# FengDushuo/BBBP-Multi-Modal-Deep-Ensemble-Framework

Measured on AMD Instinct MI355X. Metric: molecules/sec fwd+bwd (3-branch ensemble, B=512), higher is better.
Workload: dtype f32; 1 GPU; MixedInputModel F=167 (MACCS) + 3x128x128 image, 6-layer encoder + 2-stage CNN + fusion + BN head; forward + MSE + backward + fused AdamW, train mode (dropout 0.1); global_batch=512, per_gpu_batch=512, parallelism=dp1, input=device-resident

## Files before the change

bbbp-multi-modal-deep-ensemble-framework_amd/csrc/head.hip:

```cpp
#include "common.h"
#include "bbbp_hip.h"
#include "head_sync.h"

namespace {

constexpr int ROWS = 16;
constexpr int NTH = 512;
constexpr int NW = NTH / 64;
constexpr int COMB = 256, FHID = 128, NHEADS = 4, H1 = 256, H2 = 128, H3 = 64;
constexpr int LD = COMB + 4;
typedef float f32x4g __attribute__((ext_vector_type(4), aligned(4)));
static_assert(NTH >= H1, "one thread per BatchNorm column");

struct HeadParams {
    const float* comb;
    const float* fw1[NHEADS]; const float* fb1[NHEADS]; const float* fw2[NHEADS]; const float* fb2[NHEADS];
    const float* w0; const float* b0;
    const float* gamma; const float* beta; float* running_mean; float* running_var;
    const float* w3; const float* b3;
    const float* w5; const float* b5;
    const float* w7; const float* b7;
    float* hid; float* attn; float* fused; float* h; float* hb; float* bn_mean; float* bn_rstd; float* h2; float* h3; float* out;
    float* partial;
    int B, training;
    float eps, momentum;
    int concat;
    int world, rank;
};

template <int NCH>
__device__ __forceinline__ void load_b(f32x4 (&bf)[NCH], const float* Wrow ) {
#pragma unroll
    for (int c = 0; c < NCH; ++c) { f32x4g v = *reinterpret_cast<const f32x4g*>(Wrow + 16 * c); bf[c] = f32x4{v[0], v[1], v[2], v[3]}; }
}
template <int NCH>
__device__ __forceinline__ f32x4 mma_tile(const f32x4 (&af)[NCH], const f32x4 (&bf)[NCH]) {
    f32x4 acc0 = {0.f, 0.f, 0.f, 0.f}, acc1 = {0.f, 0.f, 0.f, 0.f};
#pragma unroll
    for (int c = 0; c < NCH; ++c)
#pragma unroll
        for (int j = 0; j < 4; j += 2) {
            acc0 = __builtin_amdgcn_mfma_f32_16x16x4f32(af[c][j], bf[c][j], acc0, 0, 0, 0);
            acc1 = __builtin_amdgcn_mfma_f32_16x16x4f32(af[c][j + 1], bf[c][j + 1], acc1, 0, 0, 0);
        }
    return acc0 + acc1;
}

template <int NCH>
__device__ __forceinline__ void load_a(f32x4 (&af)[NCH], const float* s, int ld, int lane) {
    const int i = lane & 15, kq = lane >> 4;
#pragma unroll
    for (int c = 0; c < NCH; ++c) af[c] = *reinterpret_cast<const f32x4*>(s + i * ld + 16 * c + 4 * kq);
}

__device__ __forceinline__ float sum16(float v) {
    v += __shfl_xor(v, 1); v += __shfl_xor(v, 2); v += __shfl_xor(v, 4); v += __shfl_xor(v, 8);
    return v;
}

__global__ __launch_bounds__(NTH) void head_a_kernel(HeadParams p) {
    __shared__ __attribute__((aligned(16))) float sC[ROWS * LD];
    __shared__ float sLogit[NW][NHEADS][ROWS];
    __shared__ float sP[ROWS][NHEADS];
    const int t = threadIdx.x, lane = t & 63, wave = t >> 6;
    const int q = lane & 15, kq = lane >> 4;
    const int r0 = blockIdx.x * ROWS, nrows = min(ROWS, p.B - r0);
    for (int idx = t; idx < ROWS * (COMB / 4); idx += NTH) {
        const int r = idx / (COMB / 4), c4 = idx % (COMB / 4);
        f32x4 v = {0.f, 0.f, 0.f, 0.f};
        if (r < nrows) v = *reinterpret_cast<const f32x4*>(p.comb + (long)(r0 + r) * COMB + c4 * 4);
        *reinterpret_cast<f32x4*>(sC + r * LD + c4 * 4) = v;
    }
    __syncthreads();
    f32x4 af[COMB / 16];
    load_a<COMB / 16>(af, sC, LD, lane);
    float lg[NHEADS][4];
    f32x4 bf[2][COMB / 16];
    const int n = wave * 16 + q;
    if (p.concat) {
        load_b<COMB / 16>(bf[0], p.w0 + (long)n * COMB + 4 * kq);
    } else {
    load_b<COMB / 16>(bf[0], p.fw1[0] + (long)n * COMB + 4 * kq);
#pragma unroll
    for (int h = 0; h < NHEADS; ++h) {
        if (h + 1 < NHEADS) load_b<COMB / 16>(bf[(h + 1) & 1], p.fw1[h + 1] + (long)n * COMB + 4 * kq);
        else load_b<COMB / 16>(bf[(h + 1) & 1], p.w0 + (long)n * COMB + 4 * kq);
        f32x4 acc = mma_tile<COMB / 16>(af, bf[h & 1]);
        const float b = p.fb1[h][n], w2 = p.fw2[h][n];
#pragma unroll
        for (int r = 0; r < 4; ++r) {
            const int row = 4 * kq + r;
            const float v = tanhf(acc[r] + b);
            if (row < nrows) p.hid[((long)h * p.B + r0 + row) * FHID + n] = v;
            lg[h][r] = sum16(v * w2);
        }
    }
    if (q == 0) {
#pragma unroll
        for (int h = 0; h < NHEADS; ++h)
#pragma unroll
            for (int r = 0; r < 4; ++r) sLogit[wave][h][4 * kq + r] = lg[h][r];
    }
    __syncthreads();
    if (t < ROWS) {
        float a[NHEADS], m = -INFINITY;
#pragma unroll
        for (int h = 0; h < NHEADS; ++h) {
            float z = 0.f;
#pragma unroll
            for (int w = 0; w < NW; ++w) z += sLogit[w][h][t];
            a[h] = z + p.fb2[h][0];
            m = fmaxf(m, a[h]);
        }
        float den = 0.f;
#pragma unroll
        for (int h = 0; h < NHEADS; ++h) { a[h] = __expf(a[h] - m); den += a[h]; }
#pragma unroll
        for (int h = 0; h < NHEADS; ++h) {
            a[h] /= den;
            sP[t][h] = a[h];
            if (t < nrows) p.attn[(long)(r0 + t) * NHEADS + h] = a[h];
        }
    }
    __syncthreads();
    for (int idx = t; idx < ROWS * COMB; idx += NTH) {
        const int r = idx / COMB, c = idx % COMB;
        const float x = sC[r * LD + c];
        float s = 0.f;
#pragma unroll
        for (int h = 0; h < NHEADS; ++h) s += sP[r][h] * x;
        sC[r * LD + c] = s;
        if (r < nrows) p.fused[(long)(r0 + r) * COMB + c] = s;
    }
    __syncthreads();
    load_a<COMB / 16>(af, sC, LD, lane);
    }
#pragma unroll
    for (int tt = 0; tt < 2; ++tt) {
        const int n0 = (wave + NW * tt) * 16 + q;
        if (tt == 0) load_b<COMB / 16>(bf[1], p.w0 + (long)((wave + NW) * 16 + q) * COMB + 4 * kq);
        f32x4 acc = mma_tile<COMB / 16>(af, bf[tt & 1]);
        const float b = p.b0[n0];
        float v[4], s = 0.f;
#pragma unroll
        for (int r = 0; r < 4; ++r) {
            const int row = 4 * kq + r;
            v[r] = fmaxf(acc[r] + b, 0.f);
            if (row < nrows) { p.h[(long)(r0 + row) * H1 + n0] = v[r]; s += v[r]; }
        }
        s += __shfl_xor(s, 16); s += __shfl_xor(s, 32);
        const float mean = s / nrows;
        float m2 = 0.f;
#pragma unroll
        for (int r = 0; r < 4; ++r) if (4 * kq + r < nrows) { const float d = v[r] - mean; m2 += d * d; }
        m2 += __shfl_xor(m2, 16); m2 += __shfl_xor(m2, 32);
        if (kq == 0) {
            const long slot = (long)p.rank * gridDim.x + blockIdx.x;
            p.partial[(slot * 2 + 0) * H1 + n0] = mean;
            p.partial[(slot * 2 + 1) * H1 + n0] = m2;
        }
    }
}

__global__ __launch_bounds__(NTH) void head_b_kernel(HeadParams p) {
    __shared__ __attribute__((aligned(16))) float sA[ROWS * LD];
    __shared__ __attribute__((aligned(16))) float sB[ROWS * (H2 + 4)];
    __shared__ __attribute__((aligned(16))) float sD[ROWS * (H3 + 4)];
    __shared__ float sMean[H1], sRstd[H1];
    const int t = threadIdx.x, lane = t & 63, wave = t >> 6;
    const int q = lane & 15, kq = lane >> 4;
    const int r0 = blockIdx.x * ROWS, nrows = min(ROWS, p.B - r0);
    const int nblocks = (p.B + ROWS - 1) / ROWS;
    f32x4 bf3[H1 / 16];
    load_b<H1 / 16>(bf3, p.w3 + (long)(wave * 16 + q) * H1 + 4 * kq);
    if (t < H1) {
        const int c = t;
        float mean, rstd;
        if (p.training) {
            float na = 0.f, ma = 0.f, m2a = 0.f;
            for (int b = 0; b < nblocks * p.world; ++b) {
                const float nb = (float)min(ROWS, p.B - (b % nblocks) * ROWS);
                const float mb = p.partial[((long)b * 2 + 0) * H1 + c], m2b = p.partial[((long)b * 2 + 1) * H1 + c];
                const float d = mb - ma, n = na + nb;
                ma += d * (nb / n);
                m2a += m2b + d * d * (na * nb / n);
                na = n;
            }
            const float nall = (float)p.B * (float)p.world;
            const float var = m2a / nall;
            mean = ma; rstd = rsqrtf(var + p.eps);
            if (blockIdx.x == 0) {
                p.running_mean[c] = (1.f - p.momentum) * p.running_mean[c] + p.momentum * mean;
                p.running_var[c] = (1.f - p.momentum) * p.running_var[c] + p.momentum * var * (nall / (nall - 1.f));
            }
        } else {
            mean = p.running_mean[c]; rstd = rsqrtf(p.running_var[c] + p.eps);
        }
        sMean[c] = mean; sRstd[c] = rstd;
        if (blockIdx.x == 0) { p.bn_mean[c] = mean; p.bn_rstd[c] = rstd; }
    }
    __syncthreads();
    for (int idx = t; idx < ROWS * H1; idx += NTH) {
        const int r = idx / H1, c = idx % H1;
        float v = 0.f;
        if (r < nrows) {
            v = (p.h[(long)(r0 + r) * H1 + c] - sMean[c]) * sRstd[c] * p.gamma[c] + p.beta[c];
            p.hb[(long)(r0 + r) * H1 + c] = v;
        }
        sA[r * LD + c] = v;
    }
    __syncthreads();
    {
        f32x4 af[H1 / 16];
        load_a<H1 / 16>(af, sA, LD, lane);
        const int n = wave * 16 + q;
        f32x4 acc = mma_tile<H1 / 16>(af, bf3);
        const float b = p.b3[n];
#pragma unroll
        for (int r = 0; r < 4; ++r) {
            const int row = 4 * kq + r;
            const float v = fmaxf(acc[r] + b, 0.f);
            sB[row * (H2 + 4) + n] = v;
            if (row < nrows) p.h2[(long)(r0 + row) * H2 + n] = v;
        }
    }
    __syncthreads();
    if (wave < H3 / 16) {
        f32x4 af[H2 / 16], bf[H2 / 16];
        const int n = wave * 16 + q;
        load_b<H2 / 16>(bf, p.w5 + (long)n * H2 + 4 * kq);
        load_a<H2 / 16>(af, sB, H2 + 4, lane);
        f32x4 acc = mma_tile<H2 / 16>(af, bf);
        const float b = p.b5[n];
#pragma unroll
        for (int r = 0; r < 4; ++r) {
            const int row = 4 * kq + r;
            const float v = fmaxf(acc[r] + b, 0.f);
            sD[row * (H3 + 4) + n] = v;
            if (row < nrows) p.h3[(long)(r0 + row) * H3 + n] = v;
        }
    }
    __syncthreads();
    if (wave == 0) {
        const int row = lane >> 2, part = lane & 3;
        float s = 0.f;
#pragma unroll
        for (int k = 0; k < H3 / 4; ++k) s += sD[row * (H3 + 4) + part * (H3 / 4) + k] * p.w7[part * (H3 / 4) + k];
        s += __shfl_xor(s, 1); s += __shfl_xor(s, 2);
        if (part == 0 && row < nrows) p.out[r0 + row] = s + p.b7[0];
    }
}

struct HeadBwdParams {
    const float* dout;
    const float* comb; const float* hid; const float* attn; const float* h; const float* h2; const float* h3;
    const float* bn_mean; const float* bn_rstd; const float* gamma;
    const float* fw1[NHEADS]; const float* fw2[NHEADS];
    const float* w0; const float* w3; const float* w5; const float* w7;
    float* dh3; float* dh2; float* dhb; float* dh; float* dlogit; float* dpre; float* dcomb;
    float* dgamma; float* dbeta;
    float* partial;
    int B, training;
    int world, rank;
};

typedef float f32x2g __attribute__((ext_vector_type(2), aligned(4)));

template <int K, int T>
__device__ __forceinline__ void mma_kmajor(f32x4 (&acc)[T], const float* sA, int lda, const float* W, int ldw, int colbase, int lane) {
    const int q = lane & 15, kq = lane >> 4;
    const float* wcol = W + colbase + T * q;
#pragma unroll 4
    for (int c = 0; c < K / 16; ++c) {
        const f32x4 a = *reinterpret_cast<const f32x4*>(sA + q * lda + 16 * c + 4 * kq);
#pragma unroll
        for (int j = 0; j < 4; ++j) {
            const float* wr = wcol + (long)(16 * c + 4 * kq + j) * ldw;
            if constexpr (T == 2) {
                const f32x2g b = *reinterpret_cast<const f32x2g*>(wr);
                acc[0] = __builtin_amdgcn_mfma_f32_16x16x4f32(a[j], b[0], acc[0], 0, 0, 0);
                acc[1] = __builtin_amdgcn_mfma_f32_16x16x4f32(a[j], b[1], acc[1], 0, 0, 0);
            } else {
                acc[0] = __builtin_amdgcn_mfma_f32_16x16x4f32(a[j], wr[0], acc[0], 0, 0, 0);
            }
        }
    }
}

constexpr int LD2 = H2 + 4, LD3 = H3 + 4, LDP = FHID + 4;

__global__ __launch_bounds__(NTH) void head_bwd_a_kernel(HeadBwdParams p) {
    __shared__ __attribute__((aligned(16))) float sD3[ROWS * LD3];
    __shared__ __attribute__((aligned(16))) float sD2[ROWS * LD2];
    __shared__ float sPa[4][H1], sPb[4][H1];
    const int t = threadIdx.x, lane = t & 63, wave = t >> 6;
    const int q = lane & 15, kq = lane >> 4;
    const int r0 = blockIdx.x * ROWS, nrows = min(ROWS, p.B - r0);
    for (int idx = t; idx < ROWS * H3; idx += NTH) {
        const int r = idx / H3, c = idx % H3;
        float v = 0.f;
        if (r < nrows) {
            v = p.h3[(long)(r0 + r) * H3 + c] > 0.f ? p.dout[r0 + r] * p.w7[c] : 0.f;
            p.dh3[(long)(r0 + r) * H3 + c] = v;
        }
        sD3[r * LD3 + c] = v;
    }
    __syncthreads();
    {
        f32x4 acc[1] = {{0.f, 0.f, 0.f, 0.f}};
        mma_kmajor<H3, 1>(acc, sD3, LD3, p.w5, H2, wave * 16, lane);
        const int n = wave * 16 + q;
#pragma unroll
        for (int r = 0; r < 4; ++r) {
            const int row = 4 * kq + r;
            float v = 0.f;
            if (row < nrows) {
                v = p.h2[(long)(r0 + row) * H2 + n] > 0.f ? acc[0][r] : 0.f;
                p.dh2[(long)(r0 + row) * H2 + n] = v;
            }
            sD2[row * LD2 + n] = v;
        }
    }
    __syncthreads();
    {
        f32x4 acc[2] = {{0.f, 0.f, 0.f, 0.f}, {0.f, 0.f, 0.f, 0.f}};
        mma_kmajor<H2, 2>(acc, sD2, LD2, p.w3, H1, wave * 32, lane);
#pragma unroll
        for (int u = 0; u < 2; ++u) {
            const int n = wave * 32 + 2 * q + u;
            const float mu = p.bn_mean[n], rs = p.bn_rstd[n];
            float pa = 0.f, pb = 0.f;
#pragma unroll
            for (int r = 0; r < 4; ++r) {
                const int row = 4 * kq + r;
                if (row < nrows) {
                    const float g = acc[u][r];
                    p.dhb[(long)(r0 + row) * H1 + n] = g;
                    pa += g * (p.h[(long)(r0 + row) * H1 + n] - mu) * rs;
                    pb += g;
                }
            }
            sPa[kq][n] = pa; sPb[kq][n] = pb;
        }
    }
    __syncthreads();
    if (t < H1) {
        const long slot = (long)p.rank * gridDim.x + blockIdx.x;
        p.partial[(slot * 2 + 0) * H1 + t] = ((sPa[0][t] + sPa[1][t]) + sPa[2][t]) + sPa[3][t];
        p.partial[(slot * 2 + 1) * H1 + t] = ((sPb[0][t] + sPb[1][t]) + sPb[2][t]) + sPb[3][t];
    }
}

__global__ __launch_bounds__(NTH) void head_bwd_c_kernel(HeadBwdParams p) {
    __shared__ __attribute__((aligned(16))) float sX[ROWS * LD];
    __shared__ __attribute__((aligned(16))) float sP[NHEADS * ROWS * LDP];
    __shared__ float sSa[H1], sSb[H1];
    const int t = threadIdx.x, lane = t & 63, wave = t >> 6;
    const int q = lane & 15, kq = lane >> 4;
    const int r0 = blockIdx.x * ROWS, nrows = min(ROWS, p.B - r0);
    const int nblocks = (p.B + ROWS - 1) / ROWS;
    if (t < H1) {
        float sa = 0.f, sb = 0.f, la = 0.f, lb = 0.f;
        for (int b = 0; b < nblocks * p.world; ++b) {
            const float va = p.partial[((long)b * 2 + 0) * H1 + t], vb = p.partial[((long)b * 2 + 1) * H1 + t];
            sa += va; sb += vb;
            if (b / nblocks == p.rank) { la += va; lb += vb; }
        }
        sSa[t] = sa; sSb[t] = sb;
        if (blockIdx.x == 0) { p.dgamma[t] = la; p.dbeta[t] = lb; }
    }
    __syncthreads();
    for (int idx = t; idx < ROWS * H1; idx += NTH) {
        const int r = idx / H1, c = idx % H1;
        float v = 0.f;
        if (r < nrows) {
            const float d = p.dhb[(long)(r0 + r) * H1 + c], xv = p.h[(long)(r0 + r) * H1 + c];
            const float g = p.gamma[c], mu = p.bn_mean[c], rs = p.bn_rstd[c];
            const float nall = (float)p.B * (float)p.world;
            v = p.training ? g * rs * (d - sSb[c] / nall - (xv - mu) * rs * (sSa[c] / nall)) : d * g * rs;
            v = xv > 0.f ? v : 0.f;
            p.dh[(long)(r0 + r) * H1 + c] = v;
        }
        sX[r * LD + c] = v;
    }
    __syncthreads();
    f32x4 df[2] = {{0.f, 0.f, 0.f, 0.f}, {0.f, 0.f, 0.f, 0.f}};
    mma_kmajor<H1, 2>(df, sX, LD, p.w0, COMB, wave * 32, lane);
    __syncthreads();
#pragma unroll
    for (int u = 0; u < 2; ++u)
#pragma unroll
        for (int r = 0; r < 4; ++r) sX[(4 * kq + r) * LD + wave * 32 + 2 * q + u] = df[u][r];
    __syncthreads();
#pragma unroll
    for (int rr = 0; rr < 2; ++rr) {
        const int r = wave * 2 + rr;
        const bool live = r < nrows;
        float a[NHEADS], asum = 0.f;
#pragma unroll
        for (int hh = 0; hh < NHEADS; ++hh) { a[hh] = live ? p.attn[(long)(r0 + r) * NHEADS + hh] : 0.f; asum += a[hh]; }
        float tt = 0.f;
#pragma unroll
        for (int c = lane; c < COMB; c += 64) {
            const float g = sX[r * LD + c];
            tt += live ? g * p.comb[(long)(r0 + r) * COMB + c] : 0.f;
            sX[r * LD + c] = g * asum;
        }
#pragma unroll
        for (int o = 32; o > 0; o >>= 1) tt += __shfl_xor(tt, o);
#pragma unroll
        for (int hh = 0; hh < NHEADS; ++hh) {
            const float dl = a[hh] * (tt - tt * asum);
            if (lane == 0 && live) p.dlogit[(long)hh * p.B + r0 + r] = dl;
#pragma unroll
            for (int c = lane; c < FHID; c += 64) {
                float v = 0.f;
                if (live) {
                    const float y = p.hid[((long)hh * p.B + r0 + r) * FHID + c];
                    v = dl * p.fw2[hh][c] * (1.f - y * y);
                    p.dpre[((long)hh * p.B + r0 + r) * FHID + c] = v;
                }
                sP[(hh * ROWS + r) * LDP + c] = v;
            }
        }
    }
    __syncthreads();
    f32x4 acc[2] = {{0.f, 0.f, 0.f, 0.f}, {0.f, 0.f, 0.f, 0.f}};
#pragma unroll
    for (int hh = 0; hh < NHEADS; ++hh) mma_kmajor<FHID, 2>(acc, sP + hh * ROWS * LDP, LDP, p.fw1[hh], COMB, wave * 32, lane);
#pragma unroll
    for (int u = 0; u < 2; ++u) {
        const int n = wave * 32 + 2 * q + u;
#pragma unroll
        for (int r = 0; r < 4; ++r) {
            const int row = 4 * kq + r;
            if (row < nrows) {
                const float v = acc[u][r] + sX[row * LD + n];
                p.dcomb[(long)(r0 + row) * COMB + n] = p.comb[(long)(r0 + row) * COMB + n] > 0.f ? v : 0.f;
            }
        }
    }
}

}

int bbbp_head_forward_fused(hipStream_t st, const float* comb, const float* const* fw1, const float* const* fb1,
                            const float* const* fw2, const float* const* fb2, const float* w0, const float* b0, const float* gamma,
                            const float* beta, float* running_mean, float* running_var, const float* w3, const float* b3,
                            const float* w5, const float* b5, const float* w7, const float* b7, float* hid, float* attn, float* fused,
                            float* h, float* hb, float* bn_mean, float* bn_rstd, float* h2, float* h3, float* out, float* partial,
                            int B, int training, int concat) {
    return bbbp_head_forward_fused_sync(st, comb, fw1, fb1, fw2, fb2, w0, b0, gamma, beta, running_mean, running_var, w3, b3, w5, b5, w7, b7,
                                        hid, attn, fused, h, hb, bn_mean, bn_rstd, h2, h3, out, partial, B, training, concat, nullptr);
}

int bbbp_head_forward_fused_sync(hipStream_t st, const float* comb, const float* const* fw1, const float* const* fb1,
                                 const float* const* fw2, const float* const* fb2, const float* w0, const float* b0, const float* gamma,
                                 const float* beta, float* running_mean, float* running_var, const float* w3, const float* b3,
                                 const float* w5, const float* b5, const float* w7, const float* b7, float* hid, float* attn, float* fused,
                                 float* h, float* hb, float* bn_mean, float* bn_rstd, float* h2, float* h3, float* out, float* partial,
                                 int B, int training, int concat, const bbbp_head_sync* sync) {
    const int world = sync ? sync->world : 1, rank = sync ? sync->rank : 0;
    BBBP_CHECK_ARG(B >= 1, "head: empty batch");
    BBBP_CHECK_ARG(world >= 1 && rank >= 0 && rank < world, "head: rank %d of %d", rank, world);
    BBBP_CHECK_ARG(!(training && (long)B * world <= 1), "Expected more than 1 value per channel when training, got input size [%d, %d]", B, H1);
    HeadParams p;
    p.comb = comb;
    for (int i = 0; i < NHEADS; ++i) { p.fw1[i] = fw1[i]; p.fb1[i] = fb1[i]; p.fw2[i] = fw2[i]; p.fb2[i] = fb2[i]; }
    p.w0 = w0; p.b0 = b0; p.gamma = gamma; p.beta = beta; p.running_mean = running_mean; p.running_var = running_var;
    p.w3 = w3; p.b3 = b3; p.w5 = w5; p.b5 = b5; p.w7 = w7; p.b7 = b7;
    p.hid = hid; p.attn = attn; p.fused = fused; p.h = h; p.hb = hb; p.bn_mean = bn_mean; p.bn_rstd = bn_rstd; p.h2 = h2; p.h3 = h3;
    p.out = out; p.partial = partial; p.B = B; p.training = training; p.eps = 1e-5f; p.momentum = 0.1f; p.concat = concat;
    p.world = world; p.rank = rank;
    const int blocks = cdiv(B, ROWS);
    hipLaunchKernelGGL(head_a_kernel, dim3(blocks), dim3(NTH), 0, st, p);
    BBBP_CHECK_LAUNCH();
    if (sync && sync->between && training) { const int rc = sync->between(); if (rc) return rc; }
    hipLaunchKernelGGL(head_b_kernel, dim3(blocks), dim3(NTH), 0, st, p);
    BBBP_CHECK_LAUNCH();
    return BBBP_OK;
}

int bbbp_head_backward_fused(hipStream_t st, const float* dout, const float* comb, const float* hid, const float* attn, const float* h,
                             const float* h2, const float* h3, const float* bn_mean, const float* bn_rstd, const float* gamma,
                             const float* const* fw1, const float* const* fw2, const float* w0, const float* w3, const float* w5,
                             const float* w7, float* dh3, float* dh2, float* dhb, float* dh, float* dlogit, float* dpre, float* dcomb,
                             float* dgamma, float* dbeta, float* partial, int B, int training) {
    return bbbp_head_backward_fused_sync(st, dout, comb, hid, attn, h, h2, h3, bn_mean, bn_rstd, gamma, fw1, fw2, w0, w3, w5, w7, dh3, dh2, dhb, dh,
                                         dlogit, dpre, dcomb, dgamma, dbeta, partial, B, training, nullptr);
}

int bbbp_head_backward_fused_sync(hipStream_t st, const float* dout, const float* comb, const float* hid, const float* attn, const float* h,
                                  const float* h2, const float* h3, const float* bn_mean, const float* bn_rstd, const float* gamma,
                                  const float* const* fw1, const float* const* fw2, const float* w0, const float* w3, const float* w5,
                                  const float* w7, float* dh3, float* dh2, float* dhb, float* dh, float* dlogit, float* dpre, float* dcomb,
                                  float* dgamma, float* dbeta, float* partial, int B, int training, const bbbp_head_sync* sync) {
    const int world = sync ? sync->world : 1, rank = sync ? sync->rank : 0;
    BBBP_CHECK_ARG(world >= 1 && rank >= 0 && rank < world, "head backward: rank %d of %d", rank, world);
    BBBP_CHECK_ARG(B >= 1, "head backward: empty batch");
    HeadBwdParams p;
    p.dout = dout; p.comb = comb; p.hid = hid; p.attn = attn; p.h = h; p.h2 = h2; p.h3 = h3;
    p.bn_mean = bn_mean; p.bn_rstd = bn_rstd; p.gamma = gamma;
    for (int i = 0; i < NHEADS; ++i) { p.fw1[i] = fw1[i]; p.fw2[i] = fw2[i]; }
    p.w0 = w0; p.w3 = w3; p.w5 = w5; p.w7 = w7;
    p.dh3 = dh3; p.dh2 = dh2; p.dhb = dhb; p.dh = dh; p.dlogit = dlogit; p.dpre = dpre; p.dcomb = dcomb;
    p.dgamma = dgamma; p.dbeta = dbeta; p.partial = partial; p.B = B; p.training = training;
    p.world = world; p.rank = rank;
    const int blocks = cdiv(B, ROWS);
    hipLaunchKernelGGL(head_bwd_a_kernel, dim3(blocks), dim3(NTH), 0, st, p);
    BBBP_CHECK_LAUNCH();
    if (sync && sync->between && training) { const int rc = sync->between(); if (rc) return rc; }
    hipLaunchKernelGGL(head_bwd_c_kernel, dim3(blocks), dim3(NTH), 0, st, p);
    BBBP_CHECK_LAUNCH();
    return BBBP_OK;
}
```

Before: 222,200 molecules/s.

## Prefetch head weights and activations into registers ahead of barriers in head kernels

```diff
diff --git a/bbbp-multi-modal-deep-ensemble-framework_amd/csrc/head.hip b/bbbp-multi-modal-deep-ensemble-framework_amd/csrc/head.hip
--- a/bbbp-multi-modal-deep-ensemble-framework_amd/csrc/head.hip
+++ b/bbbp-multi-modal-deep-ensemble-framework_amd/csrc/head.hip
@@ -58,6 +58,7 @@
     return v;
 }
 
+template <int FORM>
 __global__ __launch_bounds__(NTH) void head_a_kernel(HeadParams p) {
     __shared__ __attribute__((aligned(16))) float sC[ROWS * LD];
     __shared__ float sLogit[NW][NHEADS][ROWS];
@@ -65,37 +66,70 @@
     const int t = threadIdx.x, lane = t & 63, wave = t >> 6;
     const int q = lane & 15, kq = lane >> 4;
     const int r0 = blockIdx.x * ROWS, nrows = min(ROWS, p.B - r0);
+    const int n = wave * 16 + q;
+    f32x4 bf[2][COMB / 16];
+    float fb1v[NHEADS], fw2v[NHEADS], fb2v[NHEADS], b0v[2];
+    if constexpr (FORM) {
+        constexpr int NC = ROWS * (COMB / 4) / NTH;
+        f32x4 cv[NC];
+#pragma unroll
+        for (int i = 0; i < NC; ++i) {
+            const int idx = t + i * NTH, r = idx / (COMB / 4), c4 = idx % (COMB / 4);
+            cv[i] = f32x4{0.f, 0.f, 0.f, 0.f};
+            if (r < nrows) cv[i] = *reinterpret_cast<const f32x4*>(p.comb + (long)(r0 + r) * COMB + c4 * 4);
+        }
+        load_b<COMB / 16>(bf[0], (p.concat ? p.w0 : p.fw1[0]) + (long)n * COMB + 4 * kq);
+        if (p.concat) {
+            load_b<COMB / 16>(bf[1], p.w0 + (long)(n + NW * 16) * COMB + 4 * kq);
+#pragma unroll
+            for (int tt = 0; tt < 2; ++tt) b0v[tt] = p.b0[n + NW * 16 * tt];
+        } else {
+#pragma unroll
+            for (int h = 0; h < NHEADS; ++h) { fb1v[h] = p.fb1[h][n]; fw2v[h] = p.fw2[h][n]; fb2v[h] = p.fb2[h][0]; }
+        }
+#pragma unroll
+        for (int i = 0; i < NC; ++i) {
+            const int idx = t + i * NTH, r = idx / (COMB / 4), c4 = idx % (COMB / 4);
+            *reinterpret_cast<f32x4*>(sC + r * LD + c4 * 4) = cv[i];
+        }
+    } else {
     for (int idx = t; idx < ROWS * (COMB / 4); idx += NTH) {
         const int r = idx / (COMB / 4), c4 = idx % (COMB / 4);
         f32x4 v = {0.f, 0.f, 0.f, 0.f};
         if (r < nrows) v = *reinterpret_cast<const f32x4*>(p.comb + (long)(r0 + r) * COMB + c4 * 4);
         *reinterpret_cast<f32x4*>(sC + r * LD + c4 * 4) = v;
     }
+    }
     __syncthreads();
     f32x4 af[COMB / 16];
     load_a<COMB / 16>(af, sC, LD, lane);
     float lg[NHEADS][4];
-    f32x4 bf[2][COMB / 16];
-    const int n = wave * 16 + q;
     if (p.concat) {
-        load_b<COMB / 16>(bf[0], p.w0 + (long)n * COMB + 4 * kq);
+        if constexpr (!FORM) load_b<COMB / 16>(bf[0], p.w0 + (long)n * COMB + 4 * kq);
     } else {
-    load_b<COMB / 16>(bf[0], p.fw1[0] + (long)n * COMB + 4 * kq);
+    if constexpr (!FORM) load_b<COMB / 16>(bf[0], p.fw1[0] + (long)n * COMB + 4 * kq);
 #pragma unroll
     for (int h = 0; h < NHEADS; ++h) {
         if (h + 1 < NHEADS) load_b<COMB / 16>(bf[(h + 1) & 1], p.fw1[h + 1] + (long)n * COMB + 4 * kq);
         else load_b<COMB / 16>(bf[(h + 1) & 1], p.w0 + (long)n * COMB + 4 * kq);
+        if constexpr (FORM) __builtin_amdgcn_sched_barrier(0);
         f32x4 acc = mma_tile<COMB / 16>(af, bf[h & 1]);
-        const float b = p.fb1[h][n], w2 = p.fw2[h][n];
+        if constexpr (FORM) if (h == NHEADS - 1) {
+            load_b<COMB / 16>(bf[1], p.w0 + (long)(n + NW * 16) * COMB + 4 * kq);
+#pragma unroll
+            for (int tt = 0; tt < 2; ++tt) b0v[tt] = p.b0[n + NW * 16 * tt];
+        }
+        const float b = FORM ? fb1v[h] : p.fb1[h][n], w2 = FORM ? fw2v[h] : p.fw2[h][n];
 #pragma unroll
         for (int r = 0; r < 4; ++r) {
             const int row = 4 * kq + r;
             const float v = tanhf(acc[r] + b);
             if (row < nrows) p.hid[((long)h * p.B + r0 + row) * FHID + n] = v;
             lg[h][r] = sum16(v * w2);
-        }
-    }
-    if (q == 0) {
+            if constexpr (FORM) if (q == 0) sLogit[wave][h][row] = lg[h][r];
+        }
+    }
+    if (!FORM && q == 0) {
 #pragma unroll
         for (int h = 0; h < NHEADS; ++h)
 #pragma unroll
@@ -109,7 +143,7 @@
             float z = 0.f;
 #pragma unroll
             for (int w = 0; w < NW; ++w) z += sLogit[w][h][t];
-            a[h] = z + p.fb2[h][0];
+            a[h] = z + (FORM ? fb2v[h] : p.fb2[h][0]);
             m = fmaxf(m, a[h]);
         }
         float den = 0.f;
@@ -138,9 +172,9 @@
 #pragma unroll
     for (int tt = 0; tt < 2; ++tt) {
         const int n0 = (wave + NW * tt) * 16 + q;
-        if (tt == 0) load_b<COMB / 16>(bf[1], p.w0 + (long)((wave + NW) * 16 + q) * COMB + 4 * kq);
+        if constexpr (!FORM) if (tt == 0) load_b<COMB / 16>(bf[1], p.w0 + (long)((wave + NW) * 16 + q) * COMB + 4 * kq);
         f32x4 acc = mma_tile<COMB / 16>(af, bf[tt & 1]);
-        const float b = p.b0[n0];
+        const float b = FORM ? b0v[tt] : p.b0[n0];
         float v[4], s = 0.f;
 #pragma unroll
         for (int r = 0; r < 4; ++r) {
@@ -162,6 +196,17 @@
     }
 }
 
+constexpr int PBF = 16, PB = 32;
+template <int N>
+__device__ __forceinline__ void load_partials(float (&va)[N], float (&vb)[N], const float* partial, int b0, int total, int c) {
+#pragma unroll
+    for (int i = 0; i < N; ++i) {
+        const int b = min(b0 + i, total - 1);
+        va[i] = partial[((long)b * 2 + 0) * H1 + c]; vb[i] = partial[((long)b * 2 + 1) * H1 + c];
+    }
+}
+
+template <int FORM>
 __global__ __launch_bounds__(NTH) void head_b_kernel(HeadParams p) {
     __shared__ __attribute__((aligned(16))) float sA[ROWS * LD];
     __shared__ __attribute__((aligned(16))) float sB[ROWS * (H2 + 4)];
@@ -171,14 +216,54 @@
     const int q = lane & 15, kq = lane >> 4;
     const int r0 = blockIdx.x * ROWS, nrows = min(ROWS, p.B - r0);
     const int nblocks = (p.B + ROWS - 1) / ROWS;
+    float mbv[PBF], m2bv[PBF];
+    if constexpr (FORM) if (t < H1 && p.training) load_partials(mbv, m2bv, p.partial, 0, nblocks * p.world, t);
     f32x4 bf3[H1 / 16];
     load_b<H1 / 16>(bf3, p.w3 + (long)(wave * 16 + q) * H1 + 4 * kq);
+    constexpr int NR = ROWS * H1 / NTH;
+    f32x4 bf5[H2 / 16];
+    float hv[NR], w7v[H3 / 4], gam = 0.f, bet = 0.f, b3v = 0.f, b5v = 0.f, b7v = 0.f, rm = 0.f, rv = 0.f;
+    if constexpr (FORM) {
+        if (wave < H3 / 16) { load_b<H2 / 16>(bf5, p.w5 + (long)(wave * 16 + q) * H2 + 4 * kq); b5v = p.b5[wave * 16 + q]; }
+        if (wave == 0) {
+#pragma unroll
+            for (int k = 0; k < H3 / 4; ++k) w7v[k] = p.w7[(lane & 3) * (H3 / 4) + k];
+            b7v = p.b7[0];
+        }
+        b3v = p.b3[wave * 16 + q];
+        gam = p.gamma[t % H1]; bet = p.beta[t % H1];
+#pragma unroll
+        for (int i = 0; i < NR; ++i) {
+            const int r = t / H1 + i * (NTH / H1);
+            hv[i] = 0.f;
+            if (r < nrows) hv[i] = p.h[(long)(r0 + r) * H1 + t % H1];
+        }
+        if (t < H1 && (!p.training || blockIdx.x == 0)) { rm = p.running_mean[t]; rv = p.running_var[t]; }
+    }
     if (t < H1) {
         const int c = t;
         float mean, rstd;
         if (p.training) {
             float na = 0.f, ma = 0.f, m2a = 0.f;
-            for (int b = 0; b < nblocks * p.world; ++b) {
+            const int total = nblocks * p.world;
+            if constexpr (FORM) {
+                for (int b0 = 0; b0 < total; b0 += PBF) {
+                    if (b0 > 0) load_partials(mbv, m2bv, p.partial, b0, total, c);
+#pragma unroll
+                    for (int i = 0; i < PBF; ++i) {
+                        const int b = b0 + i;
+                        if (b < total) {
+                            const float nb = (float)min(ROWS, p.B - (b % nblocks) * ROWS);
+                            const float mb = mbv[i], m2b = m2bv[i];
+                            const float d = mb - ma, n = na + nb;
+                            ma += d * (nb / n);
+                            m2a += m2b + d * d * (na * nb / n);
+                            na = n;
+                        }
+                    }
+                }
+            } else {
+            for (int b = 0; b < total; ++b) {
                 const float nb = (float)min(ROWS, p.B - (b % nblocks) * ROWS);
                 const float mb = p.partial[((long)b * 2 + 0) * H1 + c], m2b = p.partial[((long)b * 2 + 1) * H1 + c];
                 const float d = mb - ma, n = na + nb;
@@ -186,20 +271,39 @@
                 m2a += m2b + d * d * (na * nb / n);
                 na = n;
             }
+            }
             const float nall = (float)p.B * (float)p.world;
             const float var = m2a / nall;
             mean = ma; rstd = rsqrtf(var + p.eps);
             if (blockIdx.x == 0) {
+                if constexpr (FORM) {
+#pragma clang fp contract(off)
+                    p.running_mean[c] = (1.f - p.momentum) * rm + p.momentum * mean;
+                    p.running_var[c] = __builtin_fmaf(p.momentum * var, nall / (nall - 1.f), (1.f - p.momentum) * rv);
+                } else {
                 p.running_mean[c] = (1.f - p.momentum) * p.running_mean[c] + p.momentum * mean;
                 p.running_var[c] = (1.f - p.momentum) * p.running_var[c] + p.momentum * var * (nall / (nall - 1.f));
+                }
             }
         } else {
-            mean = p.running_mean[c]; rstd = rsqrtf(p.running_var[c] + p.eps);
+            mean = FORM ? rm : p.running_mean[c]; rstd = rsqrtf((FORM ? rv : p.running_var[c]) + p.eps);
         }
         sMean[c] = mean; sRstd[c] = rstd;
         if (blockIdx.x == 0) { p.bn_mean[c] = mean; p.bn_rstd[c] = rstd; }
     }
     __syncthreads();
+    if constexpr (FORM) {
+#pragma unroll
+        for (int i = 0; i < NR; ++i) {
+            const int r = t / H1 + i * (NTH / H1), c = t % H1;
+            float v = 0.f;
+            if (r < nrows) {
+                v = (hv[i] - sMean[c]) * sRstd[c] * gam + bet;
+                p.hb[(long)(r0 + r) * H1 + c] = v;
+            }
+            sA[r * LD + c] = v;
+        }
+    } else {
     for (int idx = t; idx < ROWS * H1; idx += NTH) {
         const int r = idx / H1, c = idx % H1;
         float v = 0.f;
@@ -209,13 +313,14 @@
         }
         sA[r * LD + c] = v;
     }
+    }
     __syncthreads();
     {
         f32x4 af[H1 / 16];
         load_a<H1 / 16>(af, sA, LD, lane);
         const int n = wave * 16 + q;
         f32x4 acc = mma_tile<H1 / 16>(af, bf3);
-        const float b = p.b3[n];
+        const float b = FORM ? b3v : p.b3[n];
 #pragma unroll
         for (int r = 0; r < 4; ++r) {
             const int row = 4 * kq + r;
@@ -226,12 +331,12 @@
     }
     __syncthreads();
     if (wave < H3 / 16) {
-        f32x4 af[H2 / 16], bf[H2 / 16];
+        f32x4 af[H2 / 16];
         const int n = wave * 16 + q;
-        load_b<H2 / 16>(bf, p.w5 + (long)n * H2 + 4 * kq);
+        if constexpr (!FORM) load_b<H2 / 16>(bf5, p.w5 + (long)n * H2 + 4 * kq);
         load_a<H2 / 16>(af, sB, H2 + 4, lane);
-        f32x4 acc = mma_tile<H2 / 16>(af, bf);
-        const float b = p.b5[n];
+        f32x4 acc = mma_tile<H2 / 16>(af, bf5);
+        const float b = FORM ? b5v : p.b5[n];
 #pragma unroll
         for (int r = 0; r < 4; ++r) {
             const int row = 4 * kq + r;
@@ -245,9 +350,9 @@
         const int row = lane >> 2, part = lane & 3;
         float s = 0.f;
 #pragma unroll
-        for (int k = 0; k < H3 / 4; ++k) s += sD[row * (H3 + 4) + part * (H3 / 4) + k] * p.w7[part * (H3 / 4) + k];
+        for (int k = 0; k < H3 / 4; ++k) s += sD[row * (H3 + 4) + part * (H3 / 4) + k] * (FORM ? w7v[k] : p.w7[part * (H3 / 4) + k]);
         s += __shfl_xor(s, 1); s += __shfl_xor(s, 2);
-        if (part == 0 && row < nrows) p.out[r0 + row] = s + p.b7[0];
+        if (part == 0 && row < nrows) p.out[r0 + row] = s + (FORM ? b7v : p.b7[0]);
     }
 }
 
@@ -287,8 +392,54 @@
     }
 }
 
+constexpr int KB = 64, KBL = KB / 4;
+template <int T> struct WFrag { typedef f32x2 type; };
+template <> struct WFrag<1> { typedef float type; };
+template <int T>
+__device__ __forceinline__ void load_kblock(typename WFrag<T>::type (&w)[KBL], const float* wk, int ldw) {
+#pragma unroll
+    for (int c = 0; c < KB / 16; ++c)
+#pragma unroll
+        for (int j = 0; j < 4; ++j) {
+            const float* wr = wk + (long)(16 * c + j) * ldw;
+            if constexpr (T == 2) { const f32x2g b = *reinterpret_cast<const f32x2g*>(wr); w[4 * c + j] = f32x2{b[0], b[1]}; }
+            else w[4 * c + j] = wr[0];
+        }
+}
+template <int T>
+__device__ __forceinline__ void mma_kblock(f32x4 (&acc)[T], const float* sa, const typename WFrag<T>::type (&w)[KBL]) {
+#pragma unroll
+    for (int c = 0; c < KB / 16; ++c) {
+        const f32x4 a = *reinterpret_cast<const f32x4*>(sa + 16 * c);
+#pragma unroll
+        for (int j = 0; j < 4; ++j) {
+            if constexpr (T == 2) {
+                acc[0] = __builtin_amdgcn_mfma_f32_16x16x4f32(a[j], w[4 * c + j][0], acc[0], 0, 0, 0);
+                acc[1] = __builtin_amdgcn_mfma_f32_16x16x4f32(a[j], w[4 * c + j][1], acc[1], 0, 0, 0);
+            } else {
+                acc[0] = __builtin_amdgcn_mfma_f32_16x16x4f32(a[j], w[4 * c + j], acc[0], 0, 0, 0);
+            }
+        }
+    }
+}
+template <int NKB, bool NEXT>
+__device__ __forceinline__ void mma_kmajor_blocks(f32x4 (&acc)[2], const float* sa, const float* wk, int ldw, f32x2 (&w)[2][KBL],
+                                                  const float* wk_next, int ldw_next) {
+    static_assert(NKB % 2 == 0, "the next product's first block lands in w[0]");
+#pragma unroll
+    for (int b = 0; b < NKB; ++b) {
+        __builtin_amdgcn_sched_barrier(0);
+        if (b + 1 < NKB) load_kblock<2>(w[(b + 1) & 1], wk + (long)(b + 1) * KB * ldw, ldw);
+        else if constexpr (NEXT) load_kblock<2>(w[(b + 1) & 1], wk_next, ldw_next);
+        __builtin_amdgcn_sched_barrier(0);
+        mma_kblock<2>(acc, sa + b * KB, w[b & 1]);
+    }
+    __builtin_amdgcn_sched_barrier(0);
+}
+
 constexpr int LD2 = H2 + 4, LD3 = H3 + 4, LDP = FHID + 4;
 
+template <int FORM>
 __global__ __launch_bounds__(NTH) void head_bwd_a_kernel(HeadBwdParams p) {
     __shared__ __attribute__((aligned(16))) float sD3[ROWS * LD3];
     __shared__ __attribute__((aligned(16))) float sD2[ROWS * LD2];
@@ -296,6 +447,49 @@
     const int t = threadIdx.x, lane = t & 63, wave = t >> 6;
     const int q = lane & 15, kq = lane >> 4;
     const int r0 = blockIdx.x * ROWS, nrows = min(ROWS, p.B - r0);
+    constexpr int N3 = ROWS * H3 / NTH;
+    static_assert(H3 == KB && H2 == 2 * KB, "W5 is one K block, W3 two");
+    float h3v[N3], dov[N3], w7c = 0.f, w5b[KBL], h2v[4], muv[2], rsv[2], hv[2][4];
+    f32x2 w3b[2][KBL];
+    if constexpr (FORM) {
+#pragma unroll
+        for (int i = 0; i < N3; ++i) {
+            const int r = t / H3 + i * (NTH / H3);
+            h3v[i] = dov[i] = 0.f;
+            if (r < nrows) { h3v[i] = p.h3[(long)(r0 + r) * H3 + t % H3]; dov[i] = p.dout[r0 + r]; }
+        }
+        w7c = p.w7[t % H3];
+        load_kblock<1>(w5b, p.w5 + (long)(4 * kq) * H2 + wave * 16 + q, H2);
+#pragma unroll
+        for (int r = 0; r < 4; ++r) {
+            h2v[r] = 0.f;
+            if (4 * kq + r < nrows) h2v[r] = p.h2[(long)(r0 + 4 * kq + r) * H2 + wave * 16 + q];
+        }
+#pragma unroll
+        for (int b = 0; b < 2; ++b) load_kblock<2>(w3b[b], p.w3 + (long)(b * KB + 4 * kq) * H1 + wave * 32 + 2 * q, H1);
+#pragma unroll
+        for (int u = 0; u < 2; ++u) {
+            const int n = wave * 32 + 2 * q + u;
+            muv[u] = p.bn_mean[n]; rsv[u] = p.bn_rstd[n];
+#pragma unroll
+            for (int r = 0; r < 4; ++r) {
+                hv[u][r] = 0.f;
+                if (4 * kq + r < nrows) hv[u][r] = p.h[(long)(r0 + 4 * kq + r) * H1 + n];
+            }
+        }
+    }
+    if constexpr (FORM) {
+#pragma unroll
+        for (int i = 0; i < N3; ++i) {
+            const int r = t / H3 + i * (NTH / H3), c = t % H3;
+            float v = 0.f;
+            if (r < nrows) {
+                v = h3v[i] > 0.f ? dov[i] * w7c : 0.f;
+                p.dh3[(long)(r0 + r) * H3 + c] = v;
+            }
+            sD3[r * LD3 + c] = v;
+        }
+    } else {
     for (int idx = t; idx < ROWS * H3; idx += NTH) {
         const int r = idx / H3, c = idx % H3;
         float v = 0.f;
@@ -305,17 +499,19 @@
         }
         sD3[r * LD3 + c] = v;
     }
+    }
     __syncthreads();
     {
         f32x4 acc[1] = {{0.f, 0.f, 0.f, 0.f}};
-        mma_kmajor<H3, 1>(acc, sD3, LD3, p.w5, H2, wave * 16, lane);
+        if constexpr (FORM) mma_kblock<1>(acc, sD3 + q * LD3 + 4 * kq, w5b);
+        else mma_kmajor<H3, 1>(acc, sD3, LD3, p.w5, H2, wave * 16, lane);
         const int n = wave * 16 + q;
 #pragma unroll
         for (int r = 0; r < 4; ++r) {
             const int row = 4 * kq + r;
             float v = 0.f;
             if (row < nrows) {
-                v = p.h2[(long)(r0 + row) * H2 + n] > 0.f ? acc[0][r] : 0.f;
+                v = (FORM ? h2v[r] : p.h2[(long)(r0 + row) * H2 + n]) > 0.f ? acc[0][r] : 0.f;
                 p.dh2[(long)(r0 + row) * H2 + n] = v;
             }
             sD2[row * LD2 + n] = v;
@@ -324,11 +520,16 @@
     __syncthreads();
     {
         f32x4 acc[2] = {{0.f, 0.f, 0.f, 0.f}, {0.f, 0.f, 0.f, 0.f}};
-        mma_kmajor<H2, 2>(acc, sD2, LD2, p.w3, H1, wave * 32, lane);
+        if constexpr (FORM) {
+#pragma unroll
+            for (int b = 0; b < 2; ++b) mma_kblock<2>(acc, sD2 + q * LD2 + b * KB + 4 * kq, w3b[b]);
+        } else {
+            mma_kmajor<H2, 2>(acc, sD2, LD2, p.w3, H1, wave * 32, lane);
+        }
 #pragma unroll
         for (int u = 0; u < 2; ++u) {
             const int n = wave * 32 + 2 * q + u;
-            const float mu = p.bn_mean[n], rs = p.bn_rstd[n];
+            const float mu = FORM ? muv[u] : p.bn_mean[n], rs = FORM ? rsv[u] : p.bn_rstd[n];
             float pa = 0.f, pb = 0.f;
 #pragma unroll
             for (int r = 0; r < 4; ++r) {
@@ -336,7 +537,7 @@
                 if (row < nrows) {
                     const float g = acc[u][r];
                     p.dhb[(long)(r0 + row) * H1 + n] = g;
-                    pa += g * (p.h[(long)(r0 + row) * H1 + n] - mu) * rs;
+                    pa += g * ((FORM ? hv[u][r] : p.h[(long)(r0 + row) * H1 + n]) - mu) * rs;
                     pb += g;
                 }
             }
@@ -351,6 +552,7 @@
     }
 }
 
+template <int FORM>
 __global__ __launch_bounds__(NTH) void head_bwd_c_kernel(HeadBwdParams p) {
     __shared__ __attribute__((aligned(16))) float sX[ROWS * LD];
     __shared__ __attribute__((aligned(16))) float sP[NHEADS * ROWS * LDP];
@@ -359,17 +561,68 @@
     const int q = lane & 15, kq = lane >> 4;
     const int r0 = blockIdx.x * ROWS, nrows = min(ROWS, p.B - r0);
     const int nblocks = (p.B + ROWS - 1) / ROWS;
+    constexpr int NR = ROWS * H1 / NTH;
+    static_assert(H1 % (2 * KB) == 0 && FHID % (2 * KB) == 0, "whole pairs of K blocks");
+    f32x2 wb[2][KBL];
+    const float* const sxa = sX + q * LD + 4 * kq;
+    const long wlane = (long)(4 * kq) * COMB + wave * 32 + 2 * q;
+    float dv[NR], xvv[NR], gam = 0.f, muc = 0.f, rsc = 0.f;
+    float vav[PB], vbv[PB];
+    if constexpr (FORM) {
+        if (t < H1) load_partials(vav, vbv, p.partial, 0, nblocks * p.world, t);
+        load_kblock<2>(wb[0], p.w0 + wlane, COMB);
+#pragma unroll
+        for (int i = 0; i < NR; ++i) {
+            const int r = min(t / H1 + i * (NTH / H1), nrows - 1);
+            dv[i] = p.dhb[(long)(r0 + r) * H1 + t % H1]; xvv[i] = p.h[(long)(r0 + r) * H1 + t % H1];
+        }
+        gam = p.gamma[t % H1]; muc = p.bn_mean[t % H1]; rsc = p.bn_rstd[t % H1];
+        __builtin_amdgcn_sched_barrier(0);
+    }
     if (t < H1) {
         float sa = 0.f, sb = 0.f, la = 0.f, lb = 0.f;
-        for (int b = 0; b < nblocks * p.world; ++b) {
+        const int total = nblocks * p.world;
+        if constexpr (FORM) {
+            for (int b0 = 0; b0 < total; b0 += PB) {
+                if (b0 > 0) load_partials(vav, vbv, p.partial, b0, total, t);
+#pragma unroll
+                for (int i = 0; i < PB; ++i) {
+                    const int b = b0 + i;
+                    if (b < total) {
+                        const float va = vav[i], vb = vbv[i];
+                        sa += va; sb += vb;
+                        if (b / nblocks == p.rank) { la += va; lb += vb; }
+                    }
+                }
+            }
+        } else {
+        for (int b = 0; b < total; ++b) {
             const float va = p.partial[((long)b * 2 + 0) * H1 + t], vb = p.partial[((long)b * 2 + 1) * H1 + t];
             sa += va; sb += vb;
             if (b / nblocks == p.rank) { la += va; lb += vb; }
         }
+        }
         sSa[t] = sa; sSb[t] = sb;
         if (blockIdx.x == 0) { p.dgamma[t] = la; p.dbeta[t] = lb; }
     }
     __syncthreads();
+    if constexpr (FORM) {
+#pragma unroll
+        for (int i = 0; i < NR; ++i) {
+            const int r = t / H1 + i * (NTH / H1), c = t % H1;
+            float v = 0.f;
+            if (r < nrows) {
+#pragma clang fp contract(off)
+                const float d = dv[i], xv = xvv[i];
+                const float g = gam, mu = muc, rs = rsc;
+                const float nall = (float)p.B * (float)p.world;
+                v = p.training ? g * rs * (d - sSb[c] / nall - (xv - mu) * rs * (sSa[c] / nall)) : d * g * rs;
+                v = xv > 0.f ? v : 0.f;
+                p.dh[(long)(r0 + r) * H1 + c] = v;
+            }
+            sX[r * LD + c] = v;
+        }
+    } else {
     for (int idx = t; idx < ROWS * H1; idx += NTH) {
         const int r = idx / H1, c = idx % H1;
         float v = 0.f;
@@ -383,27 +636,66 @@
         }
         sX[r * LD + c] = v;
     }
+    }
+    float av[2][NHEADS], cv[2][COMB / 64], yv[2][NHEADS][FHID / 64], f2v[NHEADS][FHID / 64];
+    if constexpr (FORM) {
+#pragma unroll
+        for (int rr = 0; rr < 2; ++rr) {
+            const int r = min(wave * 2 + rr, nrows - 1);
+#pragma unroll
+            for (int hh = 0; hh < NHEADS; ++hh) av[rr][hh] = p.attn[(long)(r0 + r) * NHEADS + hh];
+#pragma unroll
+            for (int k = 0; k < COMB / 64; ++k) cv[rr][k] = p.comb[(long)(r0 + r) * COMB + lane + 64 * k];
+#pragma unroll
+            for (int hh = 0; hh < NHEADS; ++hh)
+#pragma unroll
+                for (int k = 0; k < FHID / 64; ++k) yv[rr][hh][k] = p.hid[((long)hh * p.B + r0 + r) * FHID + lane + 64 * k];
+        }
+#pragma unroll
+        for (int hh = 0; hh < NHEADS; ++hh)
+#pragma unroll
+            for (int k = 0; k < FHID / 64; ++k) f2v[hh][k] = p.fw2[hh][lane + 64 * k];
+        __builtin_amdgcn_sched_barrier(0);
+    }
     __syncthreads();
     f32x4 df[2] = {{0.f, 0.f, 0.f, 0.f}, {0.f, 0.f, 0.f, 0.f}};
-    mma_kmajor<H1, 2>(df, sX, LD, p.w0, COMB, wave * 32, lane);
+    if constexpr (FORM) mma_kmajor_blocks<H1 / KB, true>(df, sxa, p.w0 + wlane, COMB, wb, p.fw1[0] + wlane, COMB);
+    else mma_kmajor<H1, 2>(df, sX, LD, p.w0, COMB, wave * 32, lane);
     __syncthreads();
 #pragma unroll
     for (int u = 0; u < 2; ++u)
 #pragma unroll
         for (int r = 0; r < 4; ++r) sX[(4 * kq + r) * LD + wave * 32 + 2 * q + u] = df[u][r];
     __syncthreads();
+    float cm[2][4];
+    if constexpr (FORM) {
+#pragma unroll
+        for (int u = 0; u < 2; ++u)
+#pragma unroll
+            for (int r = 0; r < 4; ++r) cm[u][r] = p.comb[(long)(r0 + min(4 * kq + r, nrows - 1)) * COMB + wave * 32 + 2 * q + u];
+        __builtin_amdgcn_sched_barrier(0);
+    }
 #pragma unroll
     for (int rr = 0; rr < 2; ++rr) {
         const int r = wave * 2 + rr;
         const bool live = r < nrows;
         float a[NHEADS], asum = 0.f;
 #pragma unroll
-        for (int hh = 0; hh < NHEADS; ++hh) { a[hh] = live ? p.attn[(long)(r0 + r) * NHEADS + hh] : 0.f; asum += a[hh]; }
+        for (int hh = 0; hh < NHEADS; ++hh) {
+            if constexpr (FORM) a[hh] = live ? av[rr][hh] : 0.f;
+            else a[hh] = live ? p.attn[(long)(r0 + r) * NHEADS + hh] : 0.f;
+            asum += a[hh];
+        }
         float tt = 0.f;
 #pragma unroll
-        for (int c = lane; c < COMB; c += 64) {
+        for (int k = 0; k < COMB / 64; ++k) {
+            const int c = lane + 64 * k;
             const float g = sX[r * LD + c];
-            tt += live ? g * p.comb[(long)(r0 + r) * COMB + c] : 0.f;
+            if constexpr (FORM) {
+#pragma clang fp contract(off)
+                tt += live ? g * cv[rr][k] : 0.f;
+            }
+            else tt += live ? g * p.comb[(long)(r0 + r) * COMB + c] : 0.f;
             sX[r * LD + c] = g * asum;
         }
 #pragma unroll
@@ -413,11 +705,12 @@
             const float dl = a[hh] * (tt - tt * asum);
             if (lane == 0 && live) p.dlogit[(long)hh * p.B + r0 + r] = dl;
 #pragma unroll
-            for (int c = lane; c < FHID; c += 64) {
+            for (int k = 0; k < FHID / 64; ++k) {
+                const int c = lane + 64 * k;
                 float v = 0.f;
                 if (live) {
-                    const float y = p.hid[((long)hh * p.B + r0 + r) * FHID + c];
-                    v = dl * p.fw2[hh][c] * (1.f - y * y);
+                    const float y = FORM ? yv[rr][hh][k] : p.hid[((long)hh * p.B + r0 + r) * FHID + c];
+                    v = dl * (FORM ? f2v[hh][k] : p.fw2[hh][c]) * (1.f - y * y);
                     p.dpre[((long)hh * p.B + r0 + r) * FHID + c] = v;
                 }
                 sP[(hh * ROWS + r) * LDP + c] = v;
@@ -427,7 +720,15 @@
     __syncthreads();
     f32x4 acc[2] = {{0.f, 0.f, 0.f, 0.f}, {0.f, 0.f, 0.f, 0.f}};
 #pragma unroll
-    for (int hh = 0; hh < NHEADS; ++hh) mma_kmajor<FHID, 2>(acc, sP + hh * ROWS * LDP, LDP, p.fw1[hh], COMB, wave * 32, lane);
+    for (int hh = 0; hh < NHEADS; ++hh) {
+        if constexpr (FORM) {
+            const float* const spa = sP + (hh * ROWS + q) * LDP + 4 * kq;
+            if (hh + 1 < NHEADS) mma_kmajor_blocks<FHID / KB, true>(acc, spa, p.fw1[hh] + wlane, COMB, wb, p.fw1[hh + 1] + wlane, COMB);
+            else mma_kmajor_blocks<FHID / KB, false>(acc, spa, p.fw1[hh] + wlane, COMB, wb, nullptr, 0);
+        } else {
+            mma_kmajor<FHID, 2>(acc, sP + hh * ROWS * LDP, LDP, p.fw1[hh], COMB, wave * 32, lane);
+        }
+    }
 #pragma unroll
     for (int u = 0; u < 2; ++u) {
         const int n = wave * 32 + 2 * q + u;
@@ -436,10 +737,15 @@
             const int row = 4 * kq + r;
             if (row < nrows) {
                 const float v = acc[u][r] + sX[row * LD + n];
-                p.dcomb[(long)(r0 + row) * COMB + n] = p.comb[(long)(r0 + row) * COMB + n] > 0.f ? v : 0.f;
-            }
-        }
-    }
+                p.dcomb[(long)(r0 + row) * COMB + n] = (FORM ? cm[u][r] : p.comb[(long)(r0 + row) * COMB + n]) > 0.f ? v : 0.f;
+            }
+        }
+    }
+}
+
+int head_form() {
+    static const int form = knob_bool(bbbp_env_int("BBBP_HEAD_FORM", 1));
+    return form;
 }
 
 }
@@ -473,10 +779,11 @@
     p.out = out; p.partial = partial; p.B = B; p.training = training; p.eps = 1e-5f; p.momentum = 0.1f; p.concat = concat;
     p.world = world; p.rank = rank;
     const int blocks = cdiv(B, ROWS);
-    hipLaunchKernelGGL(head_a_kernel, dim3(blocks), dim3(NTH), 0, st, p);
+    const bool batched = head_form() != 0;
+    hipLaunchKernelGGL(batched ? head_a_kernel<1> : head_a_kernel<0>, dim3(blocks), dim3(NTH), 0, st, p);
     BBBP_CHECK_LAUNCH();
     if (sync && sync->between && training) { const int rc = sync->between(); if (rc) return rc; }
-    hipLaunchKernelGGL(head_b_kernel, dim3(blocks), dim3(NTH), 0, st, p);
+    hipLaunchKernelGGL(batched ? head_b_kernel<1> : head_b_kernel<0>, dim3(blocks), dim3(NTH), 0, st, p);
     BBBP_CHECK_LAUNCH();
     return BBBP_OK;
 }
@@ -507,10 +814,11 @@
     p.dgamma = dgamma; p.dbeta = dbeta; p.partial = partial; p.B = B; p.training = training;
     p.world = world; p.rank = rank;
     const int blocks = cdiv(B, ROWS);
-    hipLaunchKernelGGL(head_bwd_a_kernel, dim3(blocks), dim3(NTH), 0, st, p);
+    const bool batched = head_form() != 0;
+    hipLaunchKernelGGL(batched ? head_bwd_a_kernel<1> : head_bwd_a_kernel<0>, dim3(blocks), dim3(NTH), 0, st, p);
     BBBP_CHECK_LAUNCH();
     if (sync && sync->between && training) { const int rc = sync->between(); if (rc) return rc; }
-    hipLaunchKernelGGL(head_bwd_c_kernel, dim3(blocks), dim3(NTH), 0, st, p);
+    hipLaunchKernelGGL(batched ? head_bwd_c_kernel<1> : head_bwd_c_kernel<0>, dim3(blocks), dim3(NTH), 0, st, p);
     BBBP_CHECK_LAUNCH();
     return BBBP_OK;
 }
```

After: 224,300 molecules/s (median of 6 runs). About the same (+1.0%).
